# ecmwf-ifs/ectrans

Hardware: AMD Instinct MI355X
Metric: dir+inv transform-pairs/sec, TCo1279 137L x 10 fields; spectral-norm rel-error (higher is better)
Workload: dtype f64

## Files before the change

ectrans_amd/csrc/ectrans_mi.hip:

```cpp
#include <atomic>
#include <chrono>
#include <cmath>
#include <cstdarg>
#include <cstdio>
#include <map>
#include <memory>
#include <string>
#include <vector>

#include <fcntl.h>
#include <sys/mman.h>
#include <sys/stat.h>
#include <unistd.h>

#include "../../include/ectrans_mi.h"
#include "emi_kernels.h"
#include "emi_setup.h"
#include <dlfcn.h>

struct EmiRoctx {
  int (*push)(const char *) = nullptr;
  int (*pop)() = nullptr;
  bool tried = false;
  void load() {
// ... 164 lines not shown
static int upload(const std::vector<T> &h, T **d) {
  void *p = nullptr;
  if (emi_dev_malloc(&p, h.size() * sizeof(T))) return -1;
  if ((!h.empty() && emi_h2d(p, h.data(), h.size() * sizeof(T), 0)) || emi_stream_sync(0)) {
    emi_dev_free(p);
    return -1;
  }
  *d = (T *)p;
  return 0;
}
struct DevAllocs {
  std::vector<void *> list;
  DevAllocs() = default;
  DevAllocs(const DevAllocs &) = delete;
  DevAllocs &operator=(const DevAllocs &) = delete;
  ~DevAllocs() {
    for (void *p : list) emi_dev_free(p);
  }
  int alloc(void **p, size_t bytes) {
    if (emi_dev_malloc(p, bytes)) return -1;
    list.push_back(*p);
    return 0;
  }
};
template <class T, class F>
static int upload(DevAllocs &owner, const std::vector<T> &h, F *field) {
  T *d = nullptr;
  if (upload(h, &d)) return -1;
  owner.list.push_back(d);
  *field = d;
  return 0;
}

#define EMI_LAUNCH_P(esz, kern, grid, block, lds, st, ...)                     \
  do {                                                                         \
    if ((esz) == 8) {                                                          \
      typedef double RT;                                                       \
      EMI_LAUNCH(emi_f64::kern, grid, block, lds, st, __VA_ARGS__);            \
    } else {                                                                   \
      typedef float RT;                                                        \
      EMI_LAUNCH(emi_f32::kern, grid, block, lds, st, __VA_ARGS__);            \
    }                                                                          \
  } while (0)

struct FftClass {
  int nthr = 0, fbk = 0;
  int hot = 0;
  int r16 = 0;
  int split = 0;
  int mr = 0;
  int gmem = 0;
  long long gm_elems = 0;
  std::vector<int> lats;
  int *d_lats = nullptr;
  FftRowDev *d_rows = nullptr;
  size_t lds = 0;
};
struct LegMaps {
  int2 *d_inv = nullptr, *d_dir = nullptr, *d_inv_wide = nullptr, *d_dir_wide = nullptr;
  long long n_inv = 0, n_dir = 0, n_inv_wide = 0, n_dir_wide = 0;
};

struct Plan {
  Plan() = default;
  Plan(const Plan &) = delete;
  Plan &operator=(const Plan &) = delete;
  ~Plan();
  int nsmax = 0, ndgl = 0, ndgnh = 0;
  bool reduced = false;
  bool ldll = false, shiftll = false;
  bool lam = false;
  int lam_n = 0, kdgux = 0;
  double exwn = 0.0, eywn = 0.0;
  std::vector<int> kntmp;
  std::vector<int> l_kntmp, nesm0;
  std::vector<int> l_npme;
  const int *d_npme = nullptr;
  LamDev lamdev{};
  int lam_nthr = 0;
  size_t lam_lds = 0;
  double ra = 6371229.0;
  std::vector<int> nloen, nmen, ndglu, procm;
  std::vector<int> latlo;
// ... 194 lines not shown
    const int R[3] = {A, B, C};
    for (int nt = 128; nt <= 256; nt += 64) {
      double cost = 0;
      for (int ip = 0; ip < 3; ip++) {
        if (R[ip] == 1) continue;
        const long long nb = (long long)fb * (sz / R[ip]);
        const long long sweeps = (nb + nt - 1) / nt;
        cost += (double)(sweeps * nt) / (double)nb * (mr_radix_ops(R[ip]) / R[ip] + 15.0);
      }
      cost *= 1.0 + 0.5 * (256 - nt) / 64.0;
      if (cost < best * (1.0 - 1e-9) || (cost <= best * (1.0 + 1e-9) && nt > nthr)) {
        best = cost, found = true;
        fac[0] = A, fac[1] = B, fac[2] = C, fbk = fb, nthr = nt;
      }
    }
  };
  for (int A : rs) {
    if (sz % A) continue;
    const int m1 = sz / A;
    if (m1 == 1) consider(A, 1, 1);
    for (int B : rs) {
      if (m1 % B) continue;
      const int C = m1 / B;
      if (C == 1) consider(A, B, 1);
      for (int Cc : rs)
        if (Cc == C) consider(A, B, C);
    }
  }
  return found;
}

struct FftSwitches {
  bool mr, r16, r16s, hot;
  static bool off(const char *name) { return getenv(name) && atoi(getenv(name)) == 0; }
  FftSwitches() : mr(!off("EMI_FFT_MR")), r16(!off("EMI_FFT_R16")), r16s(!off("EMI_FFT_R16S")), hot(!getenv("EMI_FFT_NO_HOT")) {}
};
struct HotPlan {
  int pc, S, nfac, fac[5], nfl;
};
static const HotPlan g_hot_plans[] = {
#define EMI_HOT_ROW(pc_, S_, nf_, a_, b_, c_, d_, e_, nfl_) {pc_, S_, nf_, {a_, b_, c_, d_, e_}, nfl_},
    EMI_HOT_PLAN_LIST(EMI_HOT_ROW)
#undef EMI_HOT_ROW
};
#define EMI_LIST_ROW(r_) r_,
static const int g_r16_list[] = {EMI_R16_LIST(EMI_LIST_ROW)}, g_r16s_list[] = {EMI_R16S_LIST(EMI_LIST_ROW)};
#undef EMI_LIST_ROW

static int fft_fields_40k(size_t per_field) {
  int fbk = 16;
  while (fbk > 1 && fbk * per_field > 40960) fbk >>= 1;
  return fbk;
}
static int fft_threads(size_t lds_bytes) { return lds_bytes <= 40960 ? 256 : (lds_bytes <= 81920 ? 512 : 1024); }

struct FftChoice {
  FftPlanDev pl{};
  int nthr = 0;
  int hot = 0;
  bool gmem = false;
};
static int fft_choose(int n, int esz, const FftSwitches &sw, FftChoice &c) {
  FftPlanDev &pl = c.pl;
  pl.n = n;
  pl.cmode = (n % 2 != 0);
  pl.sz = pl.cmode ? n : n / 2;
  std::vector<int> fac;
  pl.blue = !emi::factorize_smooth(pl.sz, fac);
  pl.S = pl.sz;
// ... 195 lines not shown
}

static int build_fft_plans(Plan &P) {
  const FftSwitches sw;
  std::map<int, int> idx;
  std::map<int, int> sidx;
  std::vector<FftShared> shared;
  FftTabSizes nt;
  P.planid.assign(P.nlat, 0);
  for (int j = 0; j < P.nlat; j++) {
    const int n = P.nloen[P.lat0 + j];
    auto it = idx.find(n);
    if (it != idx.end()) {
      P.planid[j] = it->second;
      continue;
    }
    FftChoice c;
    if (int rc = fft_choose(n, P.esz, sw, c)) return rc;
    FftPlanDev &pl = c.pl;
    const FftShared &sh = fft_share_tables(pl, sidx, shared, nt);
    pl.tw_off = sh.tw_off;
    pl.perm_off = sh.perm_off;
    for (int ip = 0; ip < pl.nfac; ip++) pl.ptw_off[ip] = sh.ptw_off[ip];
    pl.rtw_off = (int)nt.rtw;
    nt.rtw += pl.sz + 1;
    if (pl.blue) {
      pl.chirp_off = (int)nt.chirp;
      nt.chirp += pl.split ? pl.sz / 2 : pl.sz;
      pl.bhat_off = (int)nt.bhat;
      nt.bhat += pl.S;
    }
    if (nt.tw > 0x7fffffffULL || nt.ptw > 0x7fffffffULL || nt.bhat > 0x7fffffffULL) EMI_FAIL(EMI_ERR_UNSUPPORTED, "FFT tables too large");
    int cls = -1;
    for (size_t k = 0; k < P.fclass.size(); k++) {
      const FftClass &fc = P.fclass[k];
      if (fc.nthr == c.nthr && fc.fbk == pl.fbk && fc.hot == c.hot && fc.r16 == pl.r16 && fc.split == pl.split && fc.mr == pl.mr && fc.gmem == (int)c.gmem) cls = (int)k;
    }
    if (cls < 0) {
      cls = (int)P.fclass.size();
      P.fclass.emplace_back();
      FftClass &fc = P.fclass[cls];
      fc.nthr = c.nthr, fc.fbk = pl.fbk, fc.hot = c.hot, fc.r16 = pl.r16, fc.split = pl.split, fc.mr = pl.mr, fc.gmem = c.gmem;
    }
    pl.lds_class = cls;
    idx[n] = P.planid[j] = (int)P.fplans.size();
    P.fplans.push_back(pl);
  }
  if (P.lam) {
    FftPlanDev pl{};
    pl.n = pl.sz = pl.S = P.ndgl;
    pl.cmode = 1;
    std::vector<int> fac;
    pl.blue = !emi::factorize_smooth(pl.sz, fac);
    if (pl.blue) {
      pl.S = emi::next_235(2 * pl.sz - 1);
      emi::factorize_smooth(pl.S, fac);
    }
    const int fs = FFT_LDS_ELEMS(pl.S) + 1, fs_max = 160 * 1024 / (4 * P.esz);
    if (fs > fs_max || pl.S > 65535 || fac.size() > 14)
      EMI_FAIL(EMI_ERR_UNSUPPORTED,
               "ESETUP_TRANS: KDGL = %d NEEDS A WORK ARRAY OF %d COMPLEX NUMBERS PER FIELD (KDGL WHERE IT FACTORISES IN 2, 3, 5, 7, ELSE THE CONVOLUTION LENGTH ABOVE 2 KDGL); THE "
               "Y-DIRECTION KERNELS HOLD TWO FIELDS IN THE 160 KIB OF LDS: AT MOST %d",
               P.ndgl, fs, fs_max);
    pl.nfac = (int)fac.size();
    for (int i = 0; i < pl.nfac; i++) pl.fac[i] = fac[i];
    const size_t per_field = (size_t)fs * 2 * P.esz;
    pl.fbk = std::max(2, std::min(16, (int)(80 * 1024 / per_field) / 2 * 2));
    const FftShared &sh = fft_share_tables(pl, sidx, shared, nt);
    pl.tw_off = sh.tw_off;
    pl.perm_off = sh.perm_off;
    for (int ip = 0; ip < pl.nfac; ip++) pl.ptw_off[ip] = sh.ptw_off[ip];
    pl.rtw_off = (int)nt.rtw;
    nt.rtw += pl.sz + 1;
    if (pl.blue) {
      pl.chirp_off = (int)nt.chirp;
// ... 24 lines not shown
      fc.gm_elems = std::max(fc.gm_elems, (long long)pl.fbk * FFT_LDS_ELEMS(pl.S));
    else if (fc.mr)
      fc.lds = std::max(fc.lds, (size_t)pl.fbk * pl.fac[0] * ((pl.fac[1] * pl.fac[2]) | 1) * 2 * P.esz);
    else if (fc.r16)
      fc.lds = (size_t)fc.r16 * 272 * 8 + (size_t)((fc.split ? 128 * fc.r16 : 0) + 240) * 2 * P.esz;
    else
      fc.lds = std::max(fc.lds, (size_t)pl.fbk * FFT_LDS_ELEMS(pl.S) * 2 * P.esz);
  }
  std::vector<d2> tw256(15 * 16);
  for (int k1 = 1; k1 < 16; k1++)
    for (int c = 0; c < 16; c++) {
      long double a = 2.0L * (long double)M_PIl * (long double)(c * k1) / 256.0L;
      tw256[(k1 - 1) * 16 + c] = d2{(double)cosl(a), (double)-sinl(a)};
    }
  auto upload_c = [&](const std::vector<d2> &v, const void **d) {
    if (P.esz == 8) return upload(P.dev_allocs, v, d);
    std::vector<f2> w(v.size());
    for (size_t i = 0; i < v.size(); i++) w[i] = f2{(float)v[i].x, (float)v[i].y};
    return upload(P.dev_allocs, w, d);
  };
  FftTabDev &ft = P.ftab;
  if (upload_c(tw, &ft.tw) || upload_c(ptw, &ft.ptw) || upload_c(rtw, &ft.rtw) || upload_c(chirp, &ft.chirp) || upload_c(bhat, &ft.bhat) || upload_c(tw256, &ft.tw256) ||
      upload(P.dev_allocs, perm, &ft.perm) || upload(P.dev_allocs, P.fplans, &ft.plans) || upload(P.dev_allocs, P.planid, &ft.planid))
    return EMI_ERR_RUNTIME;
  for (FftClass &fc : P.fclass) {
    if (upload(P.dev_allocs, fc.lats, &fc.d_lats)) return EMI_ERR_RUNTIME;
    std::vector<FftRowDev> rows(fc.lats.size());
    for (size_t i = 0; i < fc.lats.size(); i++) {
      const int j = fc.lats[i];
      const FftPlanDev &pl = P.fplans[P.planid[j]];
      FftRowDev &r = rows[i];
      r.lat = j, r.planid = P.planid[j], r.n = pl.n, r.sz = pl.sz;
      r.nmen = P.l_nmen[j], r.fb0 = P.l_fbase[j], r.gpoff = P.l_gpoff[j], r.chirp_off = pl.chirp_off;
      r.rtw_off = pl.rtw_off, r.bhat_off = pl.bhat_off, r.ptw_off0 = pl.ptw_off[0];
      r.mr_abc = pl.mr ? (pl.fac[0] | (pl.fac[1] << 8) | (pl.fac[2] << 16) | (pl.fbk << 24)) : 0;
      r.racthe = P.racthe[P.lat0 + j], r.rw = P.rw[P.lat0 + j];
    }
    if (upload(P.dev_allocs, rows, &fc.d_rows)) return EMI_ERR_RUNTIME;
  }
  return 0;
}


struct LegpolSource {
  const char *base = nullptr;
  size_t len = 0;
  void *map = nullptr;
  size_t maplen = 0;
  std::vector<size_t> offA, offS;
  ~LegpolSource() {
    if (map) munmap(map, maplen);
  }
};

static int legpol_open(LegpolSource &src, const emi_legpol_io_t *io, bool membuf) {
  if (membuf) {
    if (!io->ptr) EMI_FAIL(EMI_ERR_ARG, "SETUP_TRANS: KLEGPOLPTR NULL POINTER");
    if (!io->len) EMI_FAIL(EMI_ERR_ARG, "SETUP_TRANS: KLEGPOLPTR_LEN ARGUMENT MISSING");
    src.base = (const char *)io->ptr;
    src.len = io->len;
    return 0;
  }
  if (!io->fname || !io->fname[0]) EMI_FAIL(EMI_ERR_ARG, "SETUP_TRANS: CDLEGPOLFNAME ARGUMENT MISSING");
  int fd = open(io->fname, O_RDONLY);
  struct stat st;
  if (fd < 0 || fstat(fd, &st) != 0) {
    if (fd >= 0) close(fd);
// ... 1220 lines not shown
    if (fc.lats.empty() || nfld <= 0) continue;
    const int nchunk = (nfld + fc.fbk - 1) / fc.fbk;
    const long long nblocks = (long long)fc.lats.size() * nchunk;
    FftLaunchDev lc{fc.d_lats, (int)fc.lats.size(), nchunk, nblocks, adj ? 1 : 0, fc.d_rows};
    const int nthr = fc.nthr;
    if (g_pt.on) g_pt.fft_kernels++;
    if (fc.gmem) {
      const size_t needb = (size_t)nblocks * fc.gm_elems * 2 * P.esz;
      if (needb > P.cap_fftscr) {
        plan_quiesce(P);
        emi_stream_sync(0);
        emi_dev_free(P.d_fftscr);
        P.d_fftscr = nullptr;
        P.cap_fftscr = 0;
        void *q = nullptr;
        if (emi_dev_malloc(&q, needb)) EMI_FAIL(EMI_ERR_RUNTIME, "cannot allocate %.2f GiB of FFT scratch for the rows that exceed the LDS", needb / 1073741824.0);
        P.d_fftscr = (char *)q;
        P.cap_fftscr = needb;
      }
      if (inverse) {
        if (P.esz == 8)
          EMI_LAUNCH(emi_f64::k_fft_inv_gm, nblocks, nthr, 0, st, P.g, P.ftab, lc, d_flds, nfld, (const double *)FB, ldf, nproma, (d2 *)P.d_fftscr, fc.gm_elems);
        else
          EMI_LAUNCH(emi_f32::k_fft_inv_gm, nblocks, nthr, 0, st, P.g, P.ftab, lc, d_flds, nfld, (const float *)FB, ldf, nproma, (f2 *)P.d_fftscr, fc.gm_elems);
      } else {
        if (P.esz == 8)
          EMI_LAUNCH(emi_f64::k_fft_dir_gm, nblocks, nthr, 0, st, P.g, P.ftab, lc, d_flds, nfld, (double *)FB, ldf, nproma, (d2 *)P.d_fftscr, fc.gm_elems);
        else
          EMI_LAUNCH(emi_f32::k_fft_dir_gm, nblocks, nthr, 0, st, P.g, P.ftab, lc, d_flds, nfld, (float *)FB, ldf, nproma, (f2 *)P.d_fftscr, fc.gm_elems);
      }
      continue;
    }
    if (fc.mr) {
      if (inverse)
        EMI_LAUNCH_P(P.esz, k_fft_inv_mr, nblocks, nthr, fc.lds, st, P.g, P.ftab, lc, d_flds, nfld, (const RT *)FB, ldf, nproma);
      else
        EMI_LAUNCH_P(P.esz, k_fft_dir_mr, nblocks, nthr, fc.lds, st, P.g, P.ftab, lc, d_flds, nfld, (RT *)FB, ldf, nproma);
      continue;
    }
    if (fc.r16 && fc.split) {
      switch (fc.r16) {
#define EMI_R16P_LAUNCH(r_)                                                                                                                 \
  case r_:                                                                                                                                  \
    if (inverse)                                                                                                                            \
      EMI_LAUNCH_P(P.esz, k_fft_inv_r16p<r_>, nblocks, nthr, fc.lds, st, P.g, P.ftab, lc, d_flds, nfld, (const RT *)FB, ldf, nproma);      \
    else                                                                                                                                    \
      EMI_LAUNCH_P(P.esz, k_fft_dir_r16p<r_>, nblocks, nthr, fc.lds, st, P.g, P.ftab, lc, d_flds, nfld, (RT *)FB, ldf, nproma);            \
    break;
        EMI_R16S_LIST(EMI_R16P_LAUNCH)
#undef EMI_R16P_LAUNCH
        default: EMI_FAIL(EMI_ERR_RUNTIME, "internal: no k_fft_*_r16p kernel for R1 = %d", fc.r16);
      }
      continue;
    }
    if (fc.r16) {
      switch (fc.r16) {
#define EMI_R16_LAUNCH(r_)                                                                                                                  \
  case r_:                                                                                                                                  \
    if (inverse)                                                                                                                            \
      EMI_LAUNCH_P(P.esz, k_fft_inv_r16<r_>, nblocks, nthr, fc.lds, st, P.g, P.ftab, lc, d_flds, nfld, (const RT *)FB, ldf, nproma);       \
    else                                                                                                                                    \
      EMI_LAUNCH_P(P.esz, k_fft_dir_r16<r_>, nblocks, nthr, fc.lds, st, P.g, P.ftab, lc, d_flds, nfld, (RT *)FB, ldf, nproma);             \
    break;
        EMI_R16_LIST(EMI_R16_LAUNCH)
#undef EMI_R16_LAUNCH
        default: EMI_FAIL(EMI_ERR_RUNTIME, "internal: no k_fft_*_r16 kernel for R1 = %d", fc.r16);
      }
      continue;
    }
    switch (fc.hot) {
// ... 83 lines not shown
      if (dcfg < 1) dcfg = 1;
    }
    return dcfg;
  }
  return cfg;
#endif
}

#ifndef EMI_CPU_EMU
static int set_lds_attrs() {
  static bool done = false;
  if (done) return 0;
  EMI_CHECK(hipFuncSetAttribute((const void *)emi_f64::k_leg_dir, hipFuncAttributeMaxDynamicSharedMemorySize, 80 * 1024));
  EMI_CHECK(hipFuncSetAttribute((const void *)emi_f32::k_leg_dir, hipFuncAttributeMaxDynamicSharedMemorySize, 80 * 1024));
#define EMI_HOT_ATTR(pc_, S_, nf_, a_, b_, c_, d_, e_, nfl_)                                                                                  \
  EMI_CHECK(hipFuncSetAttribute((const void *)emi_f64::k_fft_inv_hot<pc_>, hipFuncAttributeMaxDynamicSharedMemorySize, 160 * 1024));  \
  EMI_CHECK(hipFuncSetAttribute((const void *)emi_f64::k_fft_dir_hot<pc_>, hipFuncAttributeMaxDynamicSharedMemorySize, 160 * 1024));  \
  EMI_CHECK(hipFuncSetAttribute((const void *)emi_f32::k_fft_inv_hot<pc_>, hipFuncAttributeMaxDynamicSharedMemorySize, 160 * 1024));  \
  EMI_CHECK(hipFuncSetAttribute((const void *)emi_f32::k_fft_dir_hot<pc_>, hipFuncAttributeMaxDynamicSharedMemorySize, 160 * 1024));
  EMI_HOT_PLAN_LIST(EMI_HOT_ATTR)
#undef EMI_HOT_ATTR
  EMI_CHECK(hipFuncSetAttribute((const void *)emi_f64::k_lam_inv, hipFuncAttributeMaxDynamicSharedMemorySize, 160 * 1024));
  EMI_CHECK(hipFuncSetAttribute((const void *)emi_f64::k_lam_dir, hipFuncAttributeMaxDynamicSharedMemorySize, 160 * 1024));
  EMI_CHECK(hipFuncSetAttribute((const void *)emi_f32::k_lam_inv, hipFuncAttributeMaxDynamicSharedMemorySize, 160 * 1024));
  EMI_CHECK(hipFuncSetAttribute((const void *)emi_f32::k_lam_dir, hipFuncAttributeMaxDynamicSharedMemorySize, 160 * 1024));
  EMI_CHECK(hipFuncSetAttribute((const void *)emi_f64::k_lam_inv_ad, hipFuncAttributeMaxDynamicSharedMemorySize, 160 * 1024));
  EMI_CHECK(hipFuncSetAttribute((const void *)emi_f64::k_lam_dir_ad, hipFuncAttributeMaxDynamicSharedMemorySize, 160 * 1024));
  EMI_CHECK(hipFuncSetAttribute((const void *)emi_f32::k_lam_inv_ad, hipFuncAttributeMaxDynamicSharedMemorySize, 160 * 1024));
  EMI_CHECK(hipFuncSetAttribute((const void *)emi_f32::k_lam_dir_ad, hipFuncAttributeMaxDynamicSharedMemorySize, 160 * 1024));
  EMI_CHECK(hipFuncSetAttribute((const void *)emi_f64::k_fft_inv, hipFuncAttributeMaxDynamicSharedMemorySize, 160 * 1024));
  EMI_CHECK(hipFuncSetAttribute((const void *)emi_f64::k_fft_dir, hipFuncAttributeMaxDynamicSharedMemorySize, 160 * 1024));
  EMI_CHECK(hipFuncSetAttribute((const void *)emi_f32::k_fft_inv, hipFuncAttributeMaxDynamicSharedMemorySize, 160 * 1024));
  EMI_CHECK(hipFuncSetAttribute((const void *)emi_f32::k_fft_dir, hipFuncAttributeMaxDynamicSharedMemorySize, 160 * 1024));
  EMI_CHECK(hipFuncSetAttribute((const void *)emi_f64::k_fft_inv_mr, hipFuncAttributeMaxDynamicSharedMemorySize, 160 * 1024));
  EMI_CHECK(hipFuncSetAttribute((const void *)emi_f64::k_fft_dir_mr, hipFuncAttributeMaxDynamicSharedMemorySize, 160 * 1024));
  EMI_CHECK(hipFuncSetAttribute((const void *)emi_f32::k_fft_inv_mr, hipFuncAttributeMaxDynamicSharedMemorySize, 160 * 1024));
  EMI_CHECK(hipFuncSetAttribute((const void *)emi_f32::k_fft_dir_mr, hipFuncAttributeMaxDynamicSharedMemorySize, 160 * 1024));
#define EMI_R16_ATTR(r_)                                                                                                                     \
  EMI_CHECK(hipFuncSetAttribute((const void *)emi_f64::k_fft_inv_r16<r_>, hipFuncAttributeMaxDynamicSharedMemorySize, 160 * 1024));  \
  EMI_CHECK(hipFuncSetAttribute((const void *)emi_f64::k_fft_dir_r16<r_>, hipFuncAttributeMaxDynamicSharedMemorySize, 160 * 1024));  \
  EMI_CHECK(hipFuncSetAttribute((const void *)emi_f32::k_fft_inv_r16<r_>, hipFuncAttributeMaxDynamicSharedMemorySize, 160 * 1024));  \
  EMI_CHECK(hipFuncSetAttribute((const void *)emi_f32::k_fft_dir_r16<r_>, hipFuncAttributeMaxDynamicSharedMemorySize, 160 * 1024));
  EMI_R16_LIST(EMI_R16_ATTR)
#undef EMI_R16_ATTR
#define EMI_R16P_ATTR(r_)                                                                                                                    \
  EMI_CHECK(hipFuncSetAttribute((const void *)emi_f64::k_fft_inv_r16p<r_>, hipFuncAttributeMaxDynamicSharedMemorySize, 160 * 1024)); \
  EMI_CHECK(hipFuncSetAttribute((const void *)emi_f64::k_fft_dir_r16p<r_>, hipFuncAttributeMaxDynamicSharedMemorySize, 160 * 1024)); \
  EMI_CHECK(hipFuncSetAttribute((const void *)emi_f32::k_fft_inv_r16p<r_>, hipFuncAttributeMaxDynamicSharedMemorySize, 160 * 1024)); \
  EMI_CHECK(hipFuncSetAttribute((const void *)emi_f32::k_fft_dir_r16p<r_>, hipFuncAttributeMaxDynamicSharedMemorySize, 160 * 1024));
  EMI_R16S_LIST(EMI_R16P_ATTR)
#undef EMI_R16P_ATTR
  done = true;
  return 0;
}
#else
static int set_lds_attrs() { return 0; }
#endif

struct ScalarRef {
  int arr;
  int lev, var;
};

template <class ARGS>
static int enumerate_scalars(const ARGS &a, const char *who, std::vector<ScalarRef> &sc) {
  sc.clear();
  if (a.spscalar) {
    if (a.spsc3a || a.spsc3b || a.spsc2) EMI_FAIL(EMI_ERR_ARG, "%s : PSPSCALAR AND PSPSC3A/PSPSC3B/PSPSC2 BOTH PRESENT", who);
    for (int i = 0; i < a.nf_scalar; i++) sc.push_back({0, i, 0});
  } else {
// ... 2168 lines not shown
```

ectrans_amd/csrc/emi_mr_body.h:

```cpp

#if defined(EMI_MR_STAMP) && !defined(EMI_LEG_STAMP) && !defined(EMI_CPU_EMU)
#define MR_STAMP_BEGIN()                  \
  unsigned long long st_acc[10] = {0};    \
  unsigned long long st_prev = __builtin_readcyclecounter()
#define MR_STAMP(i_)                                                  \
  do {                                                                \
    const unsigned long long st_now = __builtin_readcyclecounter();   \
    st_acc[i_] += st_now - st_prev;                                   \
    st_prev = st_now;                                                 \
  } while (0)
#define MR_STAMP_END()                                                                \
  do {                                                                                \
    if (EMI_TID == 0) {                                                               \
      for (int i_ = 0; i_ < 10; i_++) atomicAdd(&emi_mr_stamp[i_ < 7 ? i_ : i_ + 1], st_acc[i_]); \
      atomicAdd(&emi_mr_stamp[7], 1ull);                                              \
    }                                                                                 \
  } while (0)
#else
#define MR_STAMP_BEGIN() ((void)0)
#define MR_STAMP(i_) ((void)0)
#define MR_STAMP_END() ((void)0)
#endif

template <int I, int N, class F>
// ... 107 lines not shown
        constexpr int ka = decltype(kac)::value;
        real_t ir[SB], ii[SB];
        mr_for<0, SB>([&](auto nbc) {
          constexpr int nb = decltype(nbc)::value;
          ir[nb] = tr[nb * SA + ka], ii[nb] = ti[nb * SA + ka];
        });
        MrDft<SB>::run(ir, ii, [&](auto kbc, real_t re, real_t im) {
          constexpr int kb = decltype(kbc)::value;
          emit(std::integral_constant<int, ka + SA * kb>{}, re, im);
        });
      });
    }
  }
};

EMI_DEVFN unsigned mr_magic(unsigned D) { return D > 1 ? 0xFFFFFFFFu / D + 1u : 0u; }
EMI_DEVFN unsigned mr_div(unsigned j, unsigned m) { return m ? (unsigned)(((unsigned long long)j * m) >> 32) : j; }

struct MrPassArgs {
  int cnt;
  unsigned mcnt, mD;
  int D, SU, SV, ES;
  const real2 *tw;
  int tw_by_u;
};

EMI_DEVFN real_t *mr_row(const GridFld &gf, long long blk0, unsigned rem0, int nproma) {
  return (real_t *)gf.base + (blk0 * gf.nf_arr + gf.fidx) * (long long)nproma + rem0;
}
EMI_DEVFN bool mr_row_flat(const GridFld &gf, long long blk0, unsigned rem0, int nproma, int n) {
  return (rem0 + (unsigned)n <= (unsigned)nproma) && ((((uintptr_t)mr_row(gf, blk0, rem0, nproma)) & (2 * sizeof(real_t) - 1)) == 0);
}

template <int R, int IO>
EMI_DEVFN void mr_pass(real2 *a, int fs, int nfl, const MrPassArgs &pa, const GridFld *flds, long long blk0, unsigned rem0, int nproma) {
  const int ntot = nfl * pa.cnt;
  for (int gi = EMI_TID; gi < ntot; gi += EMI_NTHREADS) {
    const int f = nfl > 1 ? (int)mr_div((unsigned)gi, pa.mcnt) : 0;
    const int j = gi - f * pa.cnt;
    const int u = pa.D > 1 ? (int)mr_div((unsigned)j, pa.mD) : j;
    const int v = j - u * pa.D;
    real2 *p = a + (long long)f * fs + u * pa.SU + v * pa.SV;
    real_t xr[R], xi[R];
    real2 w = mk2(1, 0);
    if (IO != 1 && pa.tw) {
      EMI_GLOBAL_AS const real2 *tw = (EMI_GLOBAL_AS const real2 *)pa.tw + (pa.tw_by_u ? u : j);
      w = mk2(tw->x, tw->y);
    }
    EMI_GLOBAL_AS real2 *row = nullptr;
    if constexpr (IO != 0) row = (EMI_GLOBAL_AS real2 *)mr_row(flds[f], blk0, rem0, nproma) + j;
    if constexpr (IO == 1) {
      mr_for<0, R>([&](auto rc) {
        constexpr int r = decltype(rc)::value;
        xr[r] = row[pa.cnt * r].x, xi[r] = row[pa.cnt * r].y;
      });
    } else {
      mr_for<0, R>([&](auto rc) {
        constexpr int r = decltype(rc)::value;
        const real2 z = p[r * pa.ES];
        xr[r] = z.x, xi[r] = z.y;
      });
    }
    if (IO != 1 && pa.tw) {
      if constexpr (sizeof(real_t) == 4 && (R > 8)) {
        real_t qr[4], qi[4];
        qr[1] = w.x, qi[1] = w.y;
        mr_for<1, R>([&](auto rc) {
          constexpr int r = decltype(rc)::value;
          if constexpr (r == 2) {
            qr[2] = w.x * w.x - w.y * w.y, qi[2] = 2 * w.x * w.y;
          } else if constexpr (r == 3) {
            qr[3] = qr[2] * w.x - qi[2] * w.y, qi[3] = qr[2] * w.y + qi[2] * w.x;
          } else if constexpr (r == 4) {
            qr[0] = qr[2] * qr[2] - qi[2] * qi[2], qi[0] = 2 * qr[2] * qi[2];
            w = mk2(qr[0], qi[0]);
          } else if constexpr (r > 4) {
            const real_t t0 = qr[r & 3] * w.x - qi[r & 3] * w.y;
            qi[r & 3] = qr[r & 3] * w.y + qi[r & 3] * w.x, qr[r & 3] = t0;
          }
          const real_t t1 = xr[r] * qr[r & 3] - xi[r] * qi[r & 3];
          xi[r] = xr[r] * qi[r & 3] + xi[r] * qr[r & 3], xr[r] = t1;
        });
      } else {
        real_t cr = w.x, ci = w.y;
        mr_for<1, R>([&](auto rc) {
          constexpr int r = decltype(rc)::value;
          if constexpr (r > 1) {
            const real_t t0 = cr * w.x - ci * w.y;
            ci = cr * w.y + ci * w.x, cr = t0;
          }
          const real_t t1 = xr[r] * cr - xi[r] * ci;
          xi[r] = xr[r] * ci + xi[r] * cr, xr[r] = t1;
        });
      }
    }
    MrDft<R>::run(xr, xi, [&](auto kc, real_t re, real_t im) {
      constexpr int k = decltype(kc)::value;
      if constexpr (IO == 2)
        row[pa.cnt * k].x = re, row[pa.cnt * k].y = -im;
      else
        p[k * pa.ES] = mk2(re, im);
    });
  }
}

template <int IO>
EMI_DEVFN void mr_pass_any(int R, real2 *a, int fs, int nfl, const MrPassArgs &pa, const GridFld *flds, long long blk0, unsigned rem0, int nproma) {
  switch (R) {
#define EMI_MR_CASE(r_) \
  case r_: mr_pass<r_, IO>(a, fs, nfl, pa, flds, blk0, rem0, nproma); break;
    EMI_MR_RADICES(EMI_MR_CASE)
    EMI_MR_EXTRA(EMI_MR_CASE)
#undef EMI_MR_CASE
    default: break;
  }
}

struct MrGeom {
  int A, B, C, P1, fs;
};
EMI_DEVFN MrGeom mr_geom(int abc) {
  MrGeom m;
  m.A = abc & 255, m.B = (abc >> 8) & 255, m.C = (abc >> 16) & 255;
  const int bc = m.B * m.C;
  m.P1 = bc | 1;
  m.fs = m.A * m.P1;
  return m;
}
EMI_DEVFN MrPassArgs mr_args(const MrGeom &m, int ip, const real2 *tw1, const real2 *tw2) {
  MrPassArgs pa;
  if (ip == 0) {
    pa.cnt = m.B * m.C, pa.D = 1, pa.SU = 1, pa.SV = 0, pa.ES = m.P1, pa.tw = nullptr, pa.tw_by_u = 0;
  } else if (ip == 1) {
    pa.cnt = m.A * m.C, pa.D = m.C, pa.SU = m.P1, pa.SV = 1, pa.ES = m.C, pa.tw = tw1, pa.tw_by_u = 1;
  } else {
    pa.cnt = m.A * m.B, pa.D = m.A, pa.SU = m.C, pa.SV = m.P1, pa.ES = 1, pa.tw = tw2, pa.tw_by_u = 0;
  }
  pa.mcnt = mr_magic((unsigned)pa.cnt);
  pa.mD = mr_magic((unsigned)pa.D);
  return pa;
}

EMI_KERNEL_MR(4) void k_fft_dir_mr(EmiGeomDev g, FftTabDev T, FftLaunchDev Lc, const GridFld *flds, int nfld, real_t *FB, int ldf,
                                                  int nproma) {
  EMI_LDS_DECL;
  real2 *a = (real2 *)EMI_LDS_PTR;
  const int bid = (int)xcd_swizzle(EMI_BID, Lc.nblocks, 8);
  const int li = bid / Lc.nchunk;
  const FftRowDev rw_ = Lc.rows[li];
  const FftPlanDev &pl = T.plans[rw_.planid];
  const int fbk = (int)((unsigned)rw_.mr_abc >> 24);
  const int f0 = (bid - li * Lc.nchunk) * fbk;
  const int nfl = (nfld - f0) < fbk ? (nfld - f0) : fbk;
  const int n = rw_.n, sz = rw_.sz, nmen = rw_.nmen;
  const MrGeom m = mr_geom(rw_.mr_abc);
  const int fb0 = rw_.fb0;
  const int *frow = g.fftrow ? g.fftrow + fb0 : nullptr;
  const real2 *rtw = (const real2 *)T.rtw + rw_.rtw_off;
  const real2 *tw1 = (const real2 *)T.ptw + rw_.ptw_off0, *tw2 = tw1 + m.A;
  const long long gp0 = rw_.gpoff;
  const long long blk0 = gp0 / nproma;
  const unsigned rem0 = (unsigned)(gp0 - blk0 * nproma);
  bool flat = true;
  for (int fl = 0; fl < nfl; fl++) flat = flat && mr_row_flat(flds[f0 + fl], blk0, rem0, nproma, n);
  MR_STAMP_BEGIN();
  if (flat) {
    mr_pass_any<1>(m.A, a, m.fs, nfl, mr_args(m, 0, tw1, tw2), flds + f0, blk0, rem0, nproma);
    MR_STAMP(0);
  } else {
    const int bc = m.B * m.C, pad = m.P1 - bc;
    const unsigned mbc = mr_magic((unsigned)bc);
    for (int fl = 0; fl < nfl; fl++) {
      const GridRow gr = grid_row(flds[f0 + fl], gp0, nproma);
      real2 *af = a + (long long)fl * m.fs;
      for (int l = EMI_TID; l < sz; l += EMI_NTHREADS) {
        real2 z;
        if (grid_pair_ok(gr, 2u * l)) {
          z = *(const real2 *)grid_ptr(gr, 2u * l);
        } else {
          z.x = *grid_ptr(gr, 2u * l);
          z.y = *grid_ptr(gr, 2u * l + 1);
        }
        af[l + (pad && bc > 1 ? (int)mr_div((unsigned)l, mbc) * pad : 0)] = z;
      }
    }
    EMI_SYNC();
    mr_pass_any<0>(m.A, a, m.fs, nfl, mr_args(m, 0, tw1, tw2), flds + f0, blk0, rem0, nproma);
  }
  if (m.B > 1) {
    EMI_SYNC();
    MR_STAMP(1);
    mr_pass_any<0>(m.B, a, m.fs, nfl, mr_args(m, 1, tw1, tw2), flds + f0, blk0, rem0, nproma);
    MR_STAMP(2);
  }
  if (m.C > 1) {
    EMI_SYNC();
    MR_STAMP(3);
    mr_pass_any<0>(m.C, a, m.fs, nfl, mr_args(m, 2, tw1, tw2), flds + f0, blk0, rem0, nproma);
    MR_STAMP(4);
  }
  EMI_SYNC();
  MR_STAMP(5);
  {
    const int nk = nmen + 1, ntot = nfl * nk, NT = EMI_NTHREADS;
    const unsigned mnf = mr_magic((unsigned)nfl), mA = mr_magic((unsigned)m.A), mAB = mr_magic((unsigned)(m.A * m.B));
    const real_t sc0 = (real_t)0.5 * (Lc.adj ? (real_t)1.0 : (real_t)(rw_.rw / (double)n)), racthe = (real_t)rw_.racthe;
    auto pos = [&](int k) {
      const int q1 = m.A > 1 ? (int)mr_div((unsigned)k, mA) : k;
      const int k3 = (int)mr_div((unsigned)k, mAB);
      return (k - q1 * m.A) * m.P1 + (q1 - k3 * m.B) * m.C + k3;
    };
    for (int g0 = EMI_TID; g0 < ntot; g0 += 4 * NT) {
      real2 za[4], zb[4], w4[4];
      int kk[4], ff[4];
      real_t sc[4];
#pragma unroll
      for (int e = 0; e < 4; e++) {
        const int gi = g0 + e * NT;
        if (gi < ntot) {
          const int k = nfl > 1 ? (int)mr_div((unsigned)gi, mnf) : gi, fl = gi - k * nfl;
          const real2 *af = a + (long long)fl * m.fs;
          kk[e] = k, ff[e] = fl;
          w4[e] = rtw[k];
          sc[e] = sc0 * fft_dir_mode_scale(flds[f0 + fl].mode, racthe);
          za[e] = af[pos(k)], zb[e] = af[pos(k == 0 ? 0 : sz - k)];
        }
      }
#if defined(EMI_MR_STAMP) && !defined(EMI_LEG_STAMP) && !defined(EMI_CPU_EMU)
      if (w4[0].x + za[0].x + zb[0].x + sc[0] == (real_t)1.2345e300) kk[0] = 0;
      MR_STAMP(7);
#endif
#pragma unroll
      for (int e = 0; e < 4; e++) {
        if (g0 + e * NT < ntot) {
          const real2 s1 = cadd(za[e], cconj(zb[e])), d1 = csub(za[e], cconj(zb[e]));
          const real2 tt = cmuli(cmul(w4[e], d1));
          *(real2 *)(FB + (unsigned long long)(unsigned)FROW(kk[e]) * (unsigned)ldf + 2 * (f0 + ff[e])) = mk2((s1.x - tt.x) * sc[e], (s1.y - tt.y) * sc[e]);
        }
      }
      MR_STAMP(8);
    }
  }
  MR_STAMP(6);
  MR_STAMP_END();
}

EMI_KERNEL_MR(4) void k_fft_inv_mr(EmiGeomDev g, FftTabDev T, FftLaunchDev Lc, const GridFld *flds, int nfld, const real_t *FB,
                                                  int ldf, int nproma) {
  EMI_LDS_DECL;
  real2 *a = (real2 *)EMI_LDS_PTR;
  const int bid = (int)xcd_swizzle(EMI_BID, Lc.nblocks, 8);
  const int li = bid / Lc.nchunk;
  const int lat = Lc.lats[li];
  const FftPlanDev &pl = T.plans[T.planid[lat]];
  const int fbk = pl.fbk;
  const int f0 = (bid - li * Lc.nchunk) * fbk;
  const int nfl = (nfld - f0) < fbk ? (nfld - f0) : fbk;
  const int n = pl.n, sz = pl.sz, nmen = g.nmen[lat];
  MrGeom m;
  m.A = pl.fac[0], m.B = pl.fac[1], m.C = pl.fac[2];
  m.P1 = (m.B * m.C) | 1;
  m.fs = m.A * m.P1;
  const real_t racthe = (real_t)g.racthe[lat];
  const real_t adjw = (real_t)(g.rw[lat] / (double)pl.n);
  const int fb0 = g.fbase[lat];
  const int *frow = g.fftrow ? g.fftrow + fb0 : nullptr;
  const real2 *rtw = (const real2 *)T.rtw + pl.rtw_off;
  const real2 *tw1 = (const real2 *)T.ptw + pl.ptw_off[0], *tw2 = (const real2 *)T.ptw + pl.ptw_off[1];
  const long long gp0 = g.gpoff[lat];
  const long long blk0 = gp0 / nproma;
  const unsigned rem0 = (unsigned)(gp0 - blk0 * nproma);
  {
    const int bc = m.B * m.C, pad = (bc > 1) ? m.P1 - bc : 0;
    const unsigned mbc = mr_magic((unsigned)bc);
    const int npair = sz / 2 + 1, ntot = nfl * npair, NT = EMI_NTHREADS;
    const unsigned mnf = mr_magic((unsigned)nfl);
    if (fbk == 1) {
      constexpr unsigned SZ2 = sizeof(real2);
      const GridFld gf = flds[f0];
      const unsigned rowb = (unsigned)ldf * (unsigned)sizeof(real_t);
      const EmiBuf b_fb = emi_buf(FB + (unsigned long long)(unsigned)fb0 * (unsigned)ldf + 2 * gf.src, (unsigned)nmen * rowb + SZ2);
      const EmiBuf b_rtw = emi_buf(rtw, (unsigned)(sz + 1) * SZ2);
      real_t fa, fb;
      fin_factors(gf.mode, racthe, fa, fb);
      const real_t fsc = Lc.adj ? adjw : (real_t)1.0;
      for (unsigned g0 = (unsigned)EMI_TID; g0 < (unsigned)npair; g0 += 4u * (unsigned)NT) {
        real2 xa[4], xb[4], w4[4];
#pragma unroll
        for (int e = 0; e < 4; e++) {
          const unsigned k = g0 + (unsigned)(e * NT), k2 = (unsigned)sz - k;
          if (!frow) {
            xa[e] = emi_buf_ld<real2>(b_fb, k * rowb, 0);
            xb[e] = emi_buf_ld<real2>(b_fb, k2 * rowb, 0);
          } else {
            const unsigned ka = k < (unsigned)nmen ? k : (unsigned)nmen, kb = k2 < (unsigned)nmen ? k2 : (unsigned)nmen;
            const real2 va = fin_raw(FB, frow[ka], ldf, gf.src), vb = fin_raw(FB, frow[kb], ldf, gf.src);
            xa[e] = k <= (unsigned)nmen ? va : mk2(0, 0);
            xb[e] = k2 <= (unsigned)nmen ? vb : mk2(0, 0);
          }
          w4[e] = emi_buf_ld<real2>(b_rtw, k * SZ2, 0);
        }
#pragma unroll
        for (int e = 0; e < 4; e++) {
          const unsigned k = g0 + (unsigned)(e * NT), k2 = (unsigned)sz - k;
          if (k < (unsigned)npair) {
            real2 zk, zk2;
            fin_pair(xa[e], xb[e], k, k2, fa, fb, fsc, cconj(w4[e]), mk2((real_t)1.0, (real_t)0.0), mk2((real_t)1.0, (real_t)0.0), zk, zk2);
            a[k + (pad ? mr_div(k, mbc) * (unsigned)pad : 0u)] = cconj(zk);
            if (k2 != k && k2 < (unsigned)sz) a[k2 + (pad ? mr_div(k2, mbc) * (unsigned)pad : 0u)] = cconj(zk2);
          }
// ... 1 lines not shown
      }
    } else
    for (int g0 = EMI_TID; g0 < ntot; g0 += 4 * NT) {
      real2 xa[4], xb[4], w4[4];
      real_t fa4[4], fb4[4];
      int kk[4], ff[4];
#pragma unroll
      for (int e = 0; e < 4; e++) {
        const int gi = g0 + e * NT;
        if (gi < ntot) {
          const int k = nfl > 1 ? (int)mr_div((unsigned)gi, mnf) : gi, fl = gi - k * nfl, k2 = sz - k;
          const GridFld gf = flds[f0 + fl];
          kk[e] = k, ff[e] = fl;
          xa[e] = (k <= nmen) ? fin_raw(FB, FROW(k), ldf, gf.src) : mk2(0, 0);
          xb[e] = (k2 <= nmen) ? fin_raw(FB, FROW(k2), ldf, gf.src) : mk2(0, 0);
          w4[e] = rtw[k];
          fin_factors(gf.mode, racthe, fa4[e], fb4[e]);
        }
      }
#pragma unroll
      for (int e = 0; e < 4; e++) {
        if (g0 + e * NT < ntot) {
          const int k = kk[e], k2 = sz - k;
          real2 *af = a + (long long)ff[e] * m.fs;
          real2 zk, zk2;
          fin_pair(xa[e], xb[e], (unsigned)k, (unsigned)k2, fa4[e], fb4[e], Lc.adj ? adjw : (real_t)1.0, cconj(w4[e]), mk2((real_t)1.0, (real_t)0.0), mk2((real_t)1.0, (real_t)0.0), zk, zk2);
          af[k + (pad ? (int)mr_div((unsigned)k, mbc) * pad : 0)] = cconj(zk);
          if (k2 != k && k2 < sz) af[k2 + (pad ? (int)mr_div((unsigned)k2, mbc) * pad : 0)] = cconj(zk2);
        }
      }
    }
  }
  EMI_SYNC();
  bool flat = true;
  for (int fl = 0; fl < nfl; fl++) flat = flat && mr_row_flat(flds[f0 + fl], blk0, rem0, nproma, n);
  const int last = m.C > 1 ? 2 : (m.B > 1 ? 1 : 0);
  if (last == 0 && flat)
    mr_pass_any<2>(m.A, a, m.fs, nfl, mr_args(m, 0, tw1, tw2), flds + f0, blk0, rem0, nproma);
  else
    mr_pass_any<0>(m.A, a, m.fs, nfl, mr_args(m, 0, tw1, tw2), flds + f0, blk0, rem0, nproma);
  if (m.B > 1) {
    EMI_SYNC();
    if (last == 1 && flat)
      mr_pass_any<2>(m.B, a, m.fs, nfl, mr_args(m, 1, tw1, tw2), flds + f0, blk0, rem0, nproma);
    else
      mr_pass_any<0>(m.B, a, m.fs, nfl, mr_args(m, 1, tw1, tw2), flds + f0, blk0, rem0, nproma);
  }
  if (m.C > 1) {
    EMI_SYNC();
    if (flat)
      mr_pass_any<2>(m.C, a, m.fs, nfl, mr_args(m, 2, tw1, tw2), flds + f0, blk0, rem0, nproma);
    else
      mr_pass_any<0>(m.C, a, m.fs, nfl, mr_args(m, 2, tw1, tw2), flds + f0, blk0, rem0, nproma);
  }
  if (!flat) {
    EMI_SYNC();
    const unsigned short *perm = T.perm + pl.perm_off;
    for (int fl = 0; fl < nfl; fl++) {
      const GridRow gr = grid_row(flds[f0 + fl], gp0, nproma);
      const real2 *af = a + (long long)fl * m.fs;
      for (int i = EMI_TID; i < sz; i += EMI_NTHREADS) {
        const real2 y = af[perm[i]];
        if (grid_pair_ok(gr, 2u * i)) {
          *(real2 *)grid_ptr(gr, 2u * i) = mk2(y.x, -y.y);
        } else {
          *grid_ptr(gr, 2u * i) = y.x;
          *grid_ptr(gr, 2u * i + 1) = -y.y;
        }
      }
    }
  }
}
```

Baseline: 2.992.

## Specialize mixed-radix FFT kernels by radix set and single-field blocks

```diff
diff --git a/ectrans_amd/csrc/ectrans_mi.hip b/ectrans_amd/csrc/ectrans_mi.hip
--- a/ectrans_amd/csrc/ectrans_mi.hip
+++ b/ectrans_amd/csrc/ectrans_mi.hip
@@ -220,6 +220,7 @@
   return 0;
 }
 
+#define EMI_MR_INSTANCES(X) X(0) X(1) X(2) X(3)
 #define EMI_LAUNCH_P(esz, kern, grid, block, lds, st, ...)                     \
   do {                                                                         \
     if ((esz) == 8) {                                                          \
@@ -237,6 +238,7 @@
   int r16 = 0;
   int split = 0;
   int mr = 0;
+  int mrset = 0;
   int gmem = 0;
   long long gm_elems = 0;
   std::vector<int> lats;
@@ -497,9 +499,11 @@
 
 struct FftSwitches {
   bool mr, r16, r16s, hot;
+  bool mr_full;
   static bool off(const char *name) { return getenv(name) && atoi(getenv(name)) == 0; }
-  FftSwitches() : mr(!off("EMI_FFT_MR")), r16(!off("EMI_FFT_R16")), r16s(!off("EMI_FFT_R16S")), hot(!getenv("EMI_FFT_NO_HOT")) {}
+  FftSwitches() : mr(!off("EMI_FFT_MR")), r16(!off("EMI_FFT_R16")), r16s(!off("EMI_FFT_R16S")), hot(!getenv("EMI_FFT_NO_HOT")), mr_full(getenv("EMI_FFT_MR_SET") && atoi(getenv("EMI_FFT_MR_SET")) == 1) {}
 };
+static int mr_radix_set(const int fac[3], const FftSwitches &sw) { return (sw.mr_full || fac[0] > 16 || fac[1] > 16 || fac[2] > 16) ? 1 : 0; }
 struct HotPlan {
   int pc, S, nfac, fac[5], nfl;
 };
@@ -761,15 +765,16 @@
     }
     if (nt.tw > 0x7fffffffULL || nt.ptw > 0x7fffffffULL || nt.bhat > 0x7fffffffULL) EMI_FAIL(EMI_ERR_UNSUPPORTED, "FFT tables too large");
     int cls = -1;
+    const int mrset = pl.mr ? mr_radix_set(pl.fac, sw) : 0;
     for (size_t k = 0; k < P.fclass.size(); k++) {
       const FftClass &fc = P.fclass[k];
-      if (fc.nthr == c.nthr && fc.fbk == pl.fbk && fc.hot == c.hot && fc.r16 == pl.r16 && fc.split == pl.split && fc.mr == pl.mr && fc.gmem == (int)c.gmem) cls = (int)k;
+      if (fc.nthr == c.nthr && fc.fbk == pl.fbk && fc.hot == c.hot && fc.r16 == pl.r16 && fc.split == pl.split && fc.mr == pl.mr && fc.mrset == mrset && fc.gmem == (int)c.gmem) cls = (int)k;
     }
     if (cls < 0) {
       cls = (int)P.fclass.size();
       P.fclass.emplace_back();
       FftClass &fc = P.fclass[cls];
-      fc.nthr = c.nthr, fc.fbk = pl.fbk, fc.hot = c.hot, fc.r16 = pl.r16, fc.split = pl.split, fc.mr = pl.mr, fc.gmem = c.gmem;
+      fc.nthr = c.nthr, fc.fbk = pl.fbk, fc.hot = c.hot, fc.r16 = pl.r16, fc.split = pl.split, fc.mr = pl.mr, fc.mrset = mrset, fc.gmem = c.gmem;
     }
     pl.lds_class = cls;
     idx[n] = P.planid[j] = (int)P.fplans.size();
@@ -860,7 +865,7 @@
       FftRowDev &r = rows[i];
       r.lat = j, r.planid = P.planid[j], r.n = pl.n, r.sz = pl.sz;
       r.nmen = P.l_nmen[j], r.fb0 = P.l_fbase[j], r.gpoff = P.l_gpoff[j], r.chirp_off = pl.chirp_off;
-      r.rtw_off = pl.rtw_off, r.bhat_off = pl.bhat_off, r.ptw_off0 = pl.ptw_off[0];
+      r.rtw_off = pl.rtw_off, r.bhat_off = pl.mr ? pl.perm_off : pl.bhat_off, r.ptw_off0 = pl.ptw_off[0];
       r.mr_abc = pl.mr ? (pl.fac[0] | (pl.fac[1] << 8) | (pl.fac[2] << 16) | (pl.fbk << 24)) : 0;
       r.racthe = P.racthe[P.lat0 + j], r.rw = P.rw[P.lat0 + j];
     }
@@ -2147,10 +2152,17 @@
       continue;
     }
     if (fc.mr) {
-      if (inverse)
-        EMI_LAUNCH_P(P.esz, k_fft_inv_mr, nblocks, nthr, fc.lds, st, P.g, P.ftab, lc, d_flds, nfld, (const RT *)FB, ldf, nproma);
-      else
-        EMI_LAUNCH_P(P.esz, k_fft_dir_mr, nblocks, nthr, fc.lds, st, P.g, P.ftab, lc, d_flds, nfld, (RT *)FB, ldf, nproma);
+      switch (2 * fc.mrset + (fc.fbk == 1 ? 1 : 0)) {
+#define EMI_MR_LAUNCH(v_)                                                                                                                      \
+  case v_:                                                                                                                                     \
+    if (inverse)                                                                                                                               \
+      EMI_LAUNCH_P(P.esz, k_fft_inv_mr<v_>, nblocks, nthr, fc.lds, st, P.g, P.ftab, lc, d_flds, nfld, (const RT *)FB, ldf, nproma); \
+    else                                                                                                                                       \
+      EMI_LAUNCH_P(P.esz, k_fft_dir_mr<v_>, nblocks, nthr, fc.lds, st, P.g, P.ftab, lc, d_flds, nfld, (RT *)FB, ldf, nproma);       \
+    break;
+        EMI_MR_INSTANCES(EMI_MR_LAUNCH)
+#undef EMI_MR_LAUNCH
+      }
       continue;
     }
     if (fc.r16 && fc.split) {
@@ -2300,10 +2312,13 @@
   EMI_CHECK(hipFuncSetAttribute((const void *)emi_f64::k_fft_dir, hipFuncAttributeMaxDynamicSharedMemorySize, 160 * 1024));
   EMI_CHECK(hipFuncSetAttribute((const void *)emi_f32::k_fft_inv, hipFuncAttributeMaxDynamicSharedMemorySize, 160 * 1024));
   EMI_CHECK(hipFuncSetAttribute((const void *)emi_f32::k_fft_dir, hipFuncAttributeMaxDynamicSharedMemorySize, 160 * 1024));
-  EMI_CHECK(hipFuncSetAttribute((const void *)emi_f64::k_fft_inv_mr, hipFuncAttributeMaxDynamicSharedMemorySize, 160 * 1024));
-  EMI_CHECK(hipFuncSetAttribute((const void *)emi_f64::k_fft_dir_mr, hipFuncAttributeMaxDynamicSharedMemorySize, 160 * 1024));
-  EMI_CHECK(hipFuncSetAttribute((const void *)emi_f32::k_fft_inv_mr, hipFuncAttributeMaxDynamicSharedMemorySize, 160 * 1024));
-  EMI_CHECK(hipFuncSetAttribute((const void *)emi_f32::k_fft_dir_mr, hipFuncAttributeMaxDynamicSharedMemorySize, 160 * 1024));
+#define EMI_MR_ATTR(v_)                                                                                                                                  \
+  EMI_CHECK(hipFuncSetAttribute((const void *)emi_f64::k_fft_inv_mr<v_>, hipFuncAttributeMaxDynamicSharedMemorySize, 160 * 1024)); \
+  EMI_CHECK(hipFuncSetAttribute((const void *)emi_f64::k_fft_dir_mr<v_>, hipFuncAttributeMaxDynamicSharedMemorySize, 160 * 1024)); \
+  EMI_CHECK(hipFuncSetAttribute((const void *)emi_f32::k_fft_inv_mr<v_>, hipFuncAttributeMaxDynamicSharedMemorySize, 160 * 1024)); \
+  EMI_CHECK(hipFuncSetAttribute((const void *)emi_f32::k_fft_dir_mr<v_>, hipFuncAttributeMaxDynamicSharedMemorySize, 160 * 1024));
+  EMI_MR_INSTANCES(EMI_MR_ATTR)
+#undef EMI_MR_ATTR
 #define EMI_R16_ATTR(r_)                                                                                                                     \
   EMI_CHECK(hipFuncSetAttribute((const void *)emi_f64::k_fft_inv_r16<r_>, hipFuncAttributeMaxDynamicSharedMemorySize, 160 * 1024));  \
   EMI_CHECK(hipFuncSetAttribute((const void *)emi_f64::k_fft_dir_r16<r_>, hipFuncAttributeMaxDynamicSharedMemorySize, 160 * 1024));  \
diff --git a/ectrans_amd/csrc/emi_mr_body.h b/ectrans_amd/csrc/emi_mr_body.h
--- a/ectrans_amd/csrc/emi_mr_body.h
+++ b/ectrans_amd/csrc/emi_mr_body.h
@@ -163,15 +163,17 @@
   return (rem0 + (unsigned)n <= (unsigned)nproma) && ((((uintptr_t)mr_row(gf, blk0, rem0, nproma)) & (2 * sizeof(real_t) - 1)) == 0);
 }
 
-template <int R, int IO>
-EMI_DEVFN void mr_pass(real2 *a, int fs, int nfl, const MrPassArgs &pa, const GridFld *flds, long long blk0, unsigned rem0, int nproma) {
-  const int ntot = nfl * pa.cnt;
+template <int R, int IO, int ONE>
+EMI_DEVFN void mr_pass(real2 *a, int fs, int nfl, const MrPassArgs &pa, const GridFld *flds, const real_t *row1, long long blk0, unsigned rem0, int nproma) {
+  constexpr unsigned SZ2 = sizeof(real2);
+  const int ntot = ONE ? pa.cnt : nfl * pa.cnt;
+  const EmiBuf b_row = emi_buf((ONE && IO != 0) ? (const void *)emi_uniform_ptr(row1) : (const void *)a, (unsigned)(pa.cnt * R) * SZ2);
   for (int gi = EMI_TID; gi < ntot; gi += EMI_NTHREADS) {
-    const int f = nfl > 1 ? (int)mr_div((unsigned)gi, pa.mcnt) : 0;
+    const int f = (!ONE && nfl > 1) ? (int)mr_div((unsigned)gi, pa.mcnt) : 0;
     const int j = gi - f * pa.cnt;
     const int u = pa.D > 1 ? (int)mr_div((unsigned)j, pa.mD) : j;
     const int v = j - u * pa.D;
-    real2 *p = a + (long long)f * fs + u * pa.SU + v * pa.SV;
+    real2 *p = a + (f * fs + u * pa.SU + v * pa.SV);
     real_t xr[R], xi[R];
     real2 w = mk2(1, 0);
     if (IO != 1 && pa.tw) {
@@ -179,8 +181,14 @@
       w = mk2(tw->x, tw->y);
     }
     EMI_GLOBAL_AS real2 *row = nullptr;
-    if constexpr (IO != 0) row = (EMI_GLOBAL_AS real2 *)mr_row(flds[f], blk0, rem0, nproma) + j;
-    if constexpr (IO == 1) {
+    if constexpr (IO != 0 && !ONE) row = (EMI_GLOBAL_AS real2 *)mr_row(flds[f], blk0, rem0, nproma) + j;
+    if constexpr (IO == 1 && ONE) {
+      mr_for<0, R>([&](auto rc) {
+        constexpr int r = decltype(rc)::value;
+        const real2 z = emi_buf_ld<real2>(b_row, (unsigned)j * SZ2, (unsigned)(pa.cnt * r) * SZ2);
+        xr[r] = z.x, xi[r] = z.y;
+      });
+    } else if constexpr (IO == 1) {
       mr_for<0, R>([&](auto rc) {
         constexpr int r = decltype(rc)::value;
         xr[r] = row[pa.cnt * r].x, xi[r] = row[pa.cnt * r].y;
@@ -227,7 +235,9 @@
     }
     MrDft<R>::run(xr, xi, [&](auto kc, real_t re, real_t im) {
       constexpr int k = decltype(kc)::value;
-      if constexpr (IO == 2)
+      if constexpr (IO == 2 && ONE)
+        emi_buf_st<real2>(b_row, (unsigned)j * SZ2, (unsigned)(pa.cnt * k) * SZ2, mk2(re, -im));
+      else if constexpr (IO == 2)
         row[pa.cnt * k].x = re, row[pa.cnt * k].y = -im;
       else
         p[k * pa.ES] = mk2(re, im);
@@ -235,11 +245,13 @@
   }
 }
 
-template <int IO>
-EMI_DEVFN void mr_pass_any(int R, real2 *a, int fs, int nfl, const MrPassArgs &pa, const GridFld *flds, long long blk0, unsigned rem0, int nproma) {
+template <int IO, int SET, int ONE>
+EMI_DEVFN void mr_pass_any(int R, real2 *a, int fs, int nfl, const MrPassArgs &pa, const GridFld *flds, const real_t *row1, long long blk0, unsigned rem0, int nproma) {
   switch (R) {
-#define EMI_MR_CASE(r_) \
-  case r_: mr_pass<r_, IO>(a, fs, nfl, pa, flds, blk0, rem0, nproma); break;
+#define EMI_MR_CASE(r_)                                                                                    \
+  case r_:                                                                                                 \
+    if constexpr (SET == 1 || r_ <= 16) mr_pass<r_, IO, ONE>(a, fs, nfl, pa, flds, row1, blk0, rem0, nproma);   \
+    break;
     EMI_MR_RADICES(EMI_MR_CASE)
     EMI_MR_EXTRA(EMI_MR_CASE)
 #undef EMI_MR_CASE
@@ -272,17 +284,28 @@
   return pa;
 }
 
+EMI_DEVFN unsigned mr_ld_u16(const EmiBuf &b, unsigned i) {
+#ifndef EMI_CPU_EMU
+  return (unsigned)(unsigned short)__builtin_amdgcn_raw_buffer_load_b16(b.r, i * 2u, 0, 0);
+#else
+  unsigned short v = 0;
+  if ((size_t)i * 2 + 2 <= b.bytes) memcpy(&v, b.p + (size_t)i * 2, 2);
+  return v;
+#endif
+}
+
+template <int V>
 EMI_KERNEL_MR(4) void k_fft_dir_mr(EmiGeomDev g, FftTabDev T, FftLaunchDev Lc, const GridFld *flds, int nfld, real_t *FB, int ldf,
                                                   int nproma) {
+  constexpr int SET = V >> 1, ONE = V & 1;
   EMI_LDS_DECL;
   real2 *a = (real2 *)EMI_LDS_PTR;
   const int bid = (int)xcd_swizzle(EMI_BID, Lc.nblocks, 8);
   const int li = bid / Lc.nchunk;
   const FftRowDev rw_ = Lc.rows[li];
-  const FftPlanDev &pl = T.plans[rw_.planid];
-  const int fbk = (int)((unsigned)rw_.mr_abc >> 24);
+  const int fbk = ONE ? 1 : (int)((unsigned)rw_.mr_abc >> 24);
   const int f0 = (bid - li * Lc.nchunk) * fbk;
-  const int nfl = (nfld - f0) < fbk ? (nfld - f0) : fbk;
+  const int nfl = ONE ? 1 : ((nfld - f0) < fbk ? (nfld - f0) : fbk);
   const int n = rw_.n, sz = rw_.sz, nmen = rw_.nmen;
   const MrGeom m = mr_geom(rw_.mr_abc);
   const int fb0 = rw_.fb0;
@@ -294,9 +317,10 @@
   const unsigned rem0 = (unsigned)(gp0 - blk0 * nproma);
   bool flat = true;
   for (int fl = 0; fl < nfl; fl++) flat = flat && mr_row_flat(flds[f0 + fl], blk0, rem0, nproma, n);
+  const real_t *row1 = ONE ? mr_row(flds[f0], blk0, rem0, nproma) : nullptr;
   MR_STAMP_BEGIN();
   if (flat) {
-    mr_pass_any<1>(m.A, a, m.fs, nfl, mr_args(m, 0, tw1, tw2), flds + f0, blk0, rem0, nproma);
+    mr_pass_any<1, SET, ONE>(m.A, a, m.fs, nfl, mr_args(m, 0, tw1, tw2), flds + f0, row1, blk0, rem0, nproma);
     MR_STAMP(0);
   } else {
     const int bc = m.B * m.C, pad = m.P1 - bc;
@@ -316,31 +340,60 @@
       }
     }
     EMI_SYNC();
-    mr_pass_any<0>(m.A, a, m.fs, nfl, mr_args(m, 0, tw1, tw2), flds + f0, blk0, rem0, nproma);
+    mr_pass_any<0, SET, ONE>(m.A, a, m.fs, nfl, mr_args(m, 0, tw1, tw2), flds + f0, row1, blk0, rem0, nproma);
   }
   if (m.B > 1) {
     EMI_SYNC();
     MR_STAMP(1);
-    mr_pass_any<0>(m.B, a, m.fs, nfl, mr_args(m, 1, tw1, tw2), flds + f0, blk0, rem0, nproma);
+    mr_pass_any<0, SET, ONE>(m.B, a, m.fs, nfl, mr_args(m, 1, tw1, tw2), flds + f0, row1, blk0, rem0, nproma);
     MR_STAMP(2);
   }
   if (m.C > 1) {
     EMI_SYNC();
     MR_STAMP(3);
-    mr_pass_any<0>(m.C, a, m.fs, nfl, mr_args(m, 2, tw1, tw2), flds + f0, blk0, rem0, nproma);
+    mr_pass_any<0, SET, ONE>(m.C, a, m.fs, nfl, mr_args(m, 2, tw1, tw2), flds + f0, row1, blk0, rem0, nproma);
     MR_STAMP(4);
   }
   EMI_SYNC();
   MR_STAMP(5);
   {
+    constexpr unsigned SZ2 = sizeof(real2);
     const int nk = nmen + 1, ntot = nfl * nk, NT = EMI_NTHREADS;
-    const unsigned mnf = mr_magic((unsigned)nfl), mA = mr_magic((unsigned)m.A), mAB = mr_magic((unsigned)(m.A * m.B));
+    const unsigned mnf = mr_magic((unsigned)nfl);
     const real_t sc0 = (real_t)0.5 * (Lc.adj ? (real_t)1.0 : (real_t)(rw_.rw / (double)n)), racthe = (real_t)rw_.racthe;
-    auto pos = [&](int k) {
-      const int q1 = m.A > 1 ? (int)mr_div((unsigned)k, mA) : k;
-      const int k3 = (int)mr_div((unsigned)k, mAB);
-      return (k - q1 * m.A) * m.P1 + (q1 - k3 * m.B) * m.C + k3;
-    };
+    const EmiBuf b_pm = emi_buf(T.perm + rw_.bhat_off, (unsigned)sz * 2u);
+    auto pos = [&](int k) { return (int)mr_ld_u16(b_pm, (unsigned)k); };
+    if constexpr (ONE) {
+      const real_t sc = sc0 * fft_dir_mode_scale(flds[f0].mode, racthe);
+      const unsigned rowb = (unsigned)ldf * (unsigned)sizeof(real_t);
+      const EmiBuf b_fb = emi_buf(FB + (unsigned long long)(unsigned)fb0 * (unsigned)ldf + 2 * f0, (unsigned)nmen * rowb + SZ2);
+      const EmiBuf b_rtw = emi_buf(rtw, (unsigned)(sz + 1) * SZ2);
+      for (int g0 = EMI_TID; g0 < nk; g0 += 4 * NT) {
+        real2 za[4], zb[4], w4[4];
+#pragma unroll
+        for (int e = 0; e < 4; e++) {
+          const int k = g0 + e * NT;
+          if (k < nk) {
+            w4[e] = emi_buf_ld<real2>(b_rtw, (unsigned)k * SZ2, 0);
+            za[e] = a[pos(k)], zb[e] = a[pos(k == 0 ? 0 : sz - k)];
+          }
+        }
+#pragma unroll
+        for (int e = 0; e < 4; e++) {
+          const int k = g0 + e * NT;
+          if (k < nk) {
+            const real2 s1 = cadd(za[e], cconj(zb[e])), d1 = csub(za[e], cconj(zb[e]));
+            const real2 tt = cmuli(cmul(w4[e], d1));
+            const real2 x = mk2((s1.x - tt.x) * sc, (s1.y - tt.y) * sc);
+            if (!frow)
+              emi_buf_st<real2>(b_fb, (unsigned)k * rowb, 0, x);
+            else
+              *(real2 *)(FB + (unsigned long long)(unsigned)frow[k] * (unsigned)ldf + 2 * f0) = x;
+          }
+        }
+      }
+      MR_STAMP(8);
+    } else
     for (int g0 = EMI_TID; g0 < ntot; g0 += 4 * NT) {
       real2 za[4], zb[4], w4[4];
       int kk[4], ff[4];
@@ -376,17 +429,19 @@
   MR_STAMP_END();
 }
 
+template <int V>
 EMI_KERNEL_MR(4) void k_fft_inv_mr(EmiGeomDev g, FftTabDev T, FftLaunchDev Lc, const GridFld *flds, int nfld, const real_t *FB,
                                                   int ldf, int nproma) {
+  constexpr int SET = V >> 1, ONE = V & 1;
   EMI_LDS_DECL;
   real2 *a = (real2 *)EMI_LDS_PTR;
   const int bid = (int)xcd_swizzle(EMI_BID, Lc.nblocks, 8);
   const int li = bid / Lc.nchunk;
   const int lat = Lc.lats[li];
   const FftPlanDev &pl = T.plans[T.planid[lat]];
-  const int fbk = pl.fbk;
+  const int fbk = ONE ? 1 : pl.fbk;
   const int f0 = (bid - li * Lc.nchunk) * fbk;
-  const int nfl = (nfld - f0) < fbk ? (nfld - f0) : fbk;
+  const int nfl = ONE ? 1 : ((nfld - f0) < fbk ? (nfld - f0) : fbk);
   const int n = pl.n, sz = pl.sz, nmen = g.nmen[lat];
   MrGeom m;
   m.A = pl.fac[0], m.B = pl.fac[1], m.C = pl.fac[2];
@@ -401,12 +456,15 @@
   const long long gp0 = g.gpoff[lat];
   const long long blk0 = gp0 / nproma;
   const unsigned rem0 = (unsigned)(gp0 - blk0 * nproma);
+  bool flat = true;
+  for (int fl = 0; fl < nfl; fl++) flat = flat && mr_row_flat(flds[f0 + fl], blk0, rem0, nproma, n);
+  const real_t *row1 = ONE ? mr_row(flds[f0], blk0, rem0, nproma) : nullptr;
   {
     const int bc = m.B * m.C, pad = (bc > 1) ? m.P1 - bc : 0;
     const unsigned mbc = mr_magic((unsigned)bc);
     const int npair = sz / 2 + 1, ntot = nfl * npair, NT = EMI_NTHREADS;
     const unsigned mnf = mr_magic((unsigned)nfl);
-    if (fbk == 1) {
+    if constexpr (ONE) {
       constexpr unsigned SZ2 = sizeof(real2);
       const GridFld gf = flds[f0];
       const unsigned rowb = (unsigned)ldf * (unsigned)sizeof(real_t);
@@ -474,26 +532,24 @@
     }
   }
   EMI_SYNC();
-  bool flat = true;
-  for (int fl = 0; fl < nfl; fl++) flat = flat && mr_row_flat(flds[f0 + fl], blk0, rem0, nproma, n);
   const int last = m.C > 1 ? 2 : (m.B > 1 ? 1 : 0);
   if (last == 0 && flat)
-    mr_pass_any<2>(m.A, a, m.fs, nfl, mr_args(m, 0, tw1, tw2), flds + f0, blk0, rem0, nproma);
+    mr_pass_any<2, SET, ONE>(m.A, a, m.fs, nfl, mr_args(m, 0, tw1, tw2), flds + f0, row1, blk0, rem0, nproma);
   else
-    mr_pass_any<0>(m.A, a, m.fs, nfl, mr_args(m, 0, tw1, tw2), flds + f0, blk0, rem0, nproma);
+    mr_pass_any<0, SET, ONE>(m.A, a, m.fs, nfl, mr_args(m, 0, tw1, tw2), flds + f0, row1, blk0, rem0, nproma);
   if (m.B > 1) {
     EMI_SYNC();
     if (last == 1 && flat)
-      mr_pass_any<2>(m.B, a, m.fs, nfl, mr_args(m, 1, tw1, tw2), flds + f0, blk0, rem0, nproma);
+      mr_pass_any<2, SET, ONE>(m.B, a, m.fs, nfl, mr_args(m, 1, tw1, tw2), flds + f0, row1, blk0, rem0, nproma);
     else
-      mr_pass_any<0>(m.B, a, m.fs, nfl, mr_args(m, 1, tw1, tw2), flds + f0, blk0, rem0, nproma);
+      mr_pass_any<0, SET, ONE>(m.B, a, m.fs, nfl, mr_args(m, 1, tw1, tw2), flds + f0, row1, blk0, rem0, nproma);
   }
   if (m.C > 1) {
     EMI_SYNC();
     if (flat)
-      mr_pass_any<2>(m.C, a, m.fs, nfl, mr_args(m, 2, tw1, tw2), flds + f0, blk0, rem0, nproma);
+      mr_pass_any<2, SET, ONE>(m.C, a, m.fs, nfl, mr_args(m, 2, tw1, tw2), flds + f0, row1, blk0, rem0, nproma);
     else
-      mr_pass_any<0>(m.C, a, m.fs, nfl, mr_args(m, 2, tw1, tw2), flds + f0, blk0, rem0, nproma);
+      mr_pass_any<0, SET, ONE>(m.C, a, m.fs, nfl, mr_args(m, 2, tw1, tw2), flds + f0, row1, blk0, rem0, nproma);
   }
   if (!flat) {
     EMI_SYNC();
```

New measurement: 3.007, median of 6. No clear change (+0.5%).
